# liu20050510/AA-CLIP-IQM

Hardware: AMD Instinct MI355X
Metric: images/sec ViT-L/14-336@518, batch 64 (higher is better)
Workload: dtype f16x2; 1 GPU; ViT-L/14-336 visual tower @518x518 with 4 tap layers (encode_image), batch 64 per GPU; global_batch=64, image=518x518, parallelism=dp1, input=batch resident in HBM, clip_weights=random fp32

## Files before the change

aa-clip-iqm_amd/aaclip_hip/_lib.py:

```python
from __future__ import annotations

import ctypes as C
import os
from typing import Optional

_HERE = os.path.dirname(os.path.abspath(__file__))
LIB_PATH = os.environ.get("AACLIP_LIB") or os.path.join(_HERE, "libaaclip_hip.so")
ABI_VERSION = 9

F32, F16, BF16, F16X2 = 0, 1, 2, 3
EXACT16_QKV, EXACT16_OUT, EXACT16_FC, EXACT16_PROJ, EXACT16_ADAPTER = 1, 2, 4, 8, 16
ACT_NONE, ACT_LEAKY, ACT_RELU = 0, 1, 2
EPI_BIAS, EPI_BIAS_GELU, EPI_BIAS_RESID, EPI_ACT_F32 = 0, 1, 2, 3
SEG_LOSS_FOCAL, SEG_LOSS_DICE0, SEG_LOSS_DICE1, SEG_LOSS_ALL = 1, 2, 4, 7

_vp, _i, _l, _f, _sz = C.c_void_p, C.c_int, C.c_long, C.c_float, C.c_size_t


class BlockWeights(C.Structure):
    _fields_ = [("struct_bytes", _sz)] + [(n, _vp) for n in (
        "ln1_w", "ln1_b", "qkv_w", "qkv_b", "out_w", "out_b", "ln2_w", "ln2_b",
        "fc_w", "fc_b", "proj_w", "proj_b", "adapter_w", "fc_w_fold", "fc_fold_s", "fc_fold_b",
        "qkv_w_fold", "qkv_fold_s", "qkv_fold_b")] + [("exact16", C.c_uint)]

# ... 11 lines not shown
    "aaclip_blocks": (_i, [_vp, C.POINTER(BlockWeights), _i, _f] + [_i] * 7 + [_vp, _sz, _vp]),
    "aaclip_blocks_to": (_i, [_vp, _vp, C.POINTER(BlockWeights), _i, _f] + [_i] * 7 + [_vp, _sz, _vp]),
    "aaclip_blocks_taps": (_i, [_vp, C.POINTER(_vp), C.POINTER(BlockWeights), _i, _f] + [_i] * 7 + [_vp, _sz, _vp]),
    "aaclip_tap_head": (_i, [_vp, _vp, _vp, _vp, _i, _vp, _vp, _vp] + [_i] * 5 + [_vp, _sz, _vp]),
    "aaclip_tap_head_keep_rows": (_i, [_vp, _vp, _vp, _vp, _i, _vp, _vp, _vp, _vp] + [_i] * 5 + [_vp, _sz, _vp]),
    "aaclip_det_head": (_i, [_vp, _vp, _vp, _vp, _i, _vp] + [_i] * 5 + [_vp, _sz, _vp]),
    "aaclip_anomaly_map": (_i, [C.POINTER(_vp), _i, _vp, _l, _vp, _i, _i, _i, _i, _i, _f, _vp, _sz, _vp]),
    "aaclip_similarity_map_train": (_i, [_vp, _vp, _l, _vp, _i, _i, _i, _i, _vp, _sz, _vp]),
    "aaclip_similarity_map_train_backward_workspace_bytes": (_sz, [_i, _i, _i]),
    "aaclip_similarity_map_train_backward": (_i, [_vp, _vp, _l, _vp, _vp, _vp, _vp, _i, _i, _i, _i, _vp, _sz, _vp]),
    "aaclip_seg_loss_workspace_bytes": (_sz, [_i]),
    "aaclip_seg_loss": (_i, [_vp, _l, _l, _vp, _i, _vp, _vp, _i, _l, _vp, _sz, _vp]),
    "aaclip_seg_loss_backward": (_i, [_vp, _l, _l, _vp, _i, _vp, _vp, _vp, _i, _l, _vp]),
    "aaclip_text_backward_workspace_bytes": (_sz, [_l, _i, _i]),
    "aaclip_gemm_wgrad": (_i, [_vp, _l, _vp, _l, _vp, _l, _i, _i, _vp, _sz, _vp]),
    "aaclip_attention_backward": (_i, [_vp, _vp, _vp, _i, _i, _i, _i, _f, _vp]),
    "aaclip_attention_backward_long_workspace_bytes": (_sz, [_i, _i, _i]),
    "aaclip_attention_backward_long": (_i, [_vp, _vp, _vp, _i, _i, _i, _i, _f, _vp, _sz, _vp]),
    "aaclip_layernorm_backward": (_i, [_vp, _vp, _vp, _vp, _vp, _l, _i, _f, _vp]),
    "aaclip_adapter_mix_backward": (_i, [_vp, _vp, _vp, _vp, _vp, _l, _i, _f, _vp]),
    "aaclip_block_backward": (_i, [_vp, C.POINTER(BlockWeights), C.POINTER(BlockWeights), _f] + [_i] * 6
                              + [_vp, _vp, _vp, _vp, _sz, _vp]),
    "aaclip_block_backward_long_workspace_bytes": (_sz, [_i, _i, _i, _i]),
    "aaclip_block_backward_long": (_i, [_vp, C.POINTER(BlockWeights), C.POINTER(BlockWeights), _f] + [_i] * 6
                                   + [_vp, _vp, _vp, _vp, _sz, _vp]),
    "aaclip_row_head_backward": (_i, [_vp] * 6 + [_i, _vp, _vp, _vp] + [_i] * 5 + [_vp, _sz, _vp]),
    "aaclip_text_embed": (_i, [_vp, _vp, _vp, _vp, _i, _i, _i, _i, _vp]),
    "aaclip_resample_ksize": (_i, [_i, _i]),
    "aaclip_resample_table": (_i, [_i, _i, _vp, _vp]),
    "aaclip_preprocess": (_i, [_vp, _i, _i, _i, _i, _vp, _vp, _vp, _vp, _vp, _vp, _vp]),
    "aaclip_row_head": (_i, [_vp, _vp, _vp, _vp, _vp, _i, _vp] + [_i] * 6 + [_vp, _sz, _vp]),
    "aaclip_layernorm": (_i, [_vp, _vp, _vp, _vp, _i, _l, _i, _f, _vp]),
    "aaclip_gemm": (_i, [_i, _i, _vp, _l, _vp, _vp, _vp, _l, _i, _i, _i, _i, _i, _f, _vp]),
    "aaclip_attention": (_i, [_i, _vp, _vp, _i, _i, _i, _i, _vp]),
    "aaclip_attention_log2q": (_i, [_i, _vp, _vp, _i, _i, _i, _i, _vp]),
    "aaclip_adapter_mix": (_i, [_vp, _vp, _l, _i, _f, _vp]),
    "aaclip_small_attention": (_i, [_i, _vp, _vp, _vp, _vp, _i, _i, _i, _i, _i, _f, _vp]),
    "aaclip_cross_rows_workspace_bytes": (_sz, [_i, _i, _i, _i]),
    "aaclip_cross_rows": (_i, [_i, _vp, _vp, _vp, _i, _i, _i, _i, _vp, _sz, _vp]),
    "aaclip_cross_rows_levels_workspace_bytes": (_sz, [_i, _i, _i, _i]),
    "aaclip_cross_rows_levels": (_i, [_i, _vp, _vp, _i, _vp, _i, _i, _i, _i, _i, _i, _l, _vp, _sz, _vp]),
    "aaclip_head_expand": (_i, [_i, _vp, _vp, _l, _i, _i, _f, _vp]),
    "aaclip_head_diag": (_i, [_vp, _vp, _l, _i, _i, _vp]),
    "aaclip_residual_layernorm": (_i, [_vp, _vp, _vp, _vp, _vp, _l, _i, _f, _vp]),
    "aaclip_combine3": (_i, [_vp, _vp, _vp, _f, _f, _f, _vp, _l, _vp]),
    "aaclip_linear_smallk": (_i, [_i, _vp, _vp, _vp, _vp, _l, _i, _i, _vp]),
    "aaclip_drop_cls_rows": (_i, [_i, _vp, _vp, _i, _i, _i, _i, _i, _vp]),
    "aaclip_iqm_map": (_i, [C.POINTER(_vp), _i, _vp, _vp, _vp, _i, _i, _i, _i, _f, _f, _vp, _sz, _vp]),
    "aaclip_set_gemm_variant": (_i, [_i]),
    "aaclip_profile_begin": (_i, [C.c_uint, _i]),
    "aaclip_profile_end": (_i, [C.POINTER(C.c_float), C.POINTER(C.c_int), _i]),
}

_lib: Optional[C.CDLL] = None


def load() -> C.CDLL:
    global _lib
    if _lib is None:
        if not os.path.exists(LIB_PATH):
            raise RuntimeError(
                f"{LIB_PATH} is missing: the AA-CLIP HIP extension has not been built "
                "(run `python -c 'import __graft_entry__ as g; g.build()'` or `make -C aa-clip-iqm_amd/csrc`). "
                "There is no PyTorch fallback for this path.")
        lib = C.CDLL(LIB_PATH)
        for name, (res, args) in SIGNATURES.items():
# ... 26 lines not shown
```

aa-clip-iqm_amd/csrc/capi.hip:

```cpp
#include <assert.h>
#include <stdio.h>
#include <stdlib.h>
#include <string.h>

#include "kernels.h"

using namespace aaclip;

static thread_local char g_err[512] = "";
static int g_ln_fold = 1;

static int fail(int code, const char* msg) {
  snprintf(g_err, sizeof(g_err), "%s", msg);
  return code;
}
#define REQUIRE(cond, msg) \
  do {                     \
    if (!(cond)) return fail(-1, msg); \
  } while (0)
#define REQUIRE_ALIGNED16(what, ...)                                            \
  do {                                                                          \
    const void* ptrs_[] = {__VA_ARGS__};                                        \
    for (const void* p_ : ptrs_)                                                \
      if ((uintptr_t)p_ & 15) return fail(-1, what ": pointers must be 16-byte aligned"); \
// ... 111 lines not shown
  l.big = l.narrow_bytes;
  l.big_bytes = wide > f32d ? wide : f32d;
  if (f32e > l.big_bytes) l.big_bytes = f32e;
  l.reserved = l.big + up256(l.big_bytes);
  l.x16 = l.reserved + up256((size_t)rows * 4);
  l.partials = l.x16 + up256((size_t)rows * D * es);
  l.rowab = l.partials + up256((size_t)rows * (D / 64 + 1) * 2 * 4);
  l.total = l.rowab + up256((size_t)rows * 2 * 4) + 4096;
  return l;
}

size_t aaclip_workspace_bytes(int dtype, long rows, int D, int F, int E) { return ws_layout(dtype, rows, D, F, E).total; }

int aaclip_layernorm(const float* x, const float* w, const float* b, void* out, int out_dtype, long rows, int D,
                     float eps, void* stream) {
  REQUIRE(x && w && b && out, "layernorm: null pointer");
  REQUIRE(dtype_ok(out_dtype), "layernorm: bad dtype");
  REQUIRE(rows > 0, "layernorm: rows must be positive");
  REQUIRE_ROW_WIDTH(D);
  launch_layernorm(out_dtype, x, w, b, out, rows, D, eps, (hipStream_t)stream);
  return finish("layernorm");
}

int aaclip_gemm(int dtype, int epi, const void* A, long lda, const void* W, const float* bias, void* out, long ldc,
                int M, int N, int K, int act, int scale_cols, float scale, void* stream) {
  REQUIRE(dtype_ok(dtype), "gemm: bad dtype");
  REQUIRE(epi >= AACLIP_EPI_BIAS && epi <= AACLIP_EPI_ACT_F32, "gemm: bad epilogue");
  GemmParams p = gemm_params(A, lda, W, bias, out, ldc, M, N, K);
  p.scale_cols = scale_cols; p.scale = scale; p.act = act;
  const char* m = gemm_check(dtype, epi, p);
  if (m) return fail(-1, m);
  launch_gemm(dtype, epi, p, (hipStream_t)stream);
  return finish("gemm");
}

static int attention_entry(int dtype, const void* qkv, void* ctx, int B, int L, int H, int causal, int log2q,
                           void* stream) {
  REQUIRE(qkv && ctx, "attention: null pointer");
  REQUIRE(B > 0 && L > 0 && H > 0, "attention: empty problem");
  REQUIRE(B <= 65535 && H <= 65535, "attention: grid limit");
  REQUIRE((long)L * 3 * 64 * H * 4 < (1L << 31), "attention: L * 3 * 64 * H * 4 must stay below 2^31 (32-bit row offsets)");
  REQUIRE((long)((L + 255) / 256) * H * B < (1L << 30), "attention: too many workgroups");
  launch_attention(dtype, qkv, ctx, B, L, H, causal, log2q, (hipStream_t)stream);
  return finish("attention");
}

int aaclip_attention(int dtype, const void* qkv, void* ctx, int B, int L, int H, int causal, void* stream) {
  REQUIRE(dtype_ok(dtype), "attention: bad dtype");
  return attention_entry(dtype, qkv, ctx, B, L, H, causal, 0, stream);
}

int aaclip_attention_log2q(int dtype, const void* qkv, void* ctx, int B, int L, int H, int causal, void* stream) {
  REQUIRE(dtype == AACLIP_F16 || dtype == AACLIP_BF16 || dtype == AACLIP_F16X2, "attention_log2q: 16-bit dtypes only");
  return attention_entry(dtype, qkv, ctx, B, L, H, causal, 1, stream);
}

int aaclip_adapter_mix(float* x, const float* a, long rows, int D, float weight, void* stream) {
  REQUIRE(x && a && rows > 0, "adapter_mix: bad arguments");
  REQUIRE_ROW_WIDTH(D);
  launch_adapter_mix(x, a, rows, D, weight, (hipStream_t)stream);
  return finish("adapter_mix");
}

int aaclip_small_attention(int kv_dtype, const float* q, const void* k, const void* v, float* out, int B, int nq, int Lk,
                           int H, int hd, float scale, void* stream) {
  REQUIRE(plain_dtype_ok(kv_dtype), "small_attention: bad dtype (fp32, fp16 or bf16)");
// ... 750 lines not shown
```

aa-clip-iqm_amd/csrc/common.h:

```cpp
#pragma once
#include <hip/hip_runtime.h>
#include <stdint.h>

typedef _Float16 f16;
typedef __bf16 bf16;

typedef _Float16 f16x8 __attribute__((ext_vector_type(8)));
typedef _Float16 f16x4 __attribute__((ext_vector_type(4)));
typedef __bf16 bf16x8 __attribute__((ext_vector_type(8)));
typedef __bf16 bf16x4 __attribute__((ext_vector_type(4)));
typedef short i16x4 __attribute__((ext_vector_type(4)));
typedef float f32x4 __attribute__((ext_vector_type(4)));
typedef float f32x16 __attribute__((ext_vector_type(16)));
typedef uint32_t u32x4 __attribute__((ext_vector_type(4)));
typedef uint32_t u32x2 __attribute__((ext_vector_type(2)));

#define AACLIP_DEV __device__ __forceinline__

template <typename T> struct Elem;
template <> struct Elem<f16> {
  typedef f16x8 vec8;
  typedef f16x4 vec4;
  static AACLIP_DEV f32x16 mma32(vec8 a, vec8 b, f32x16 c) {
    return __builtin_amdgcn_mfma_f32_32x32x16_f16(a, b, c, 0, 0, 0);
// ... 22 lines not shown
  c = __builtin_amdgcn_fmed3f(c * S, -448.f, 448.f);
  d = __builtin_amdgcn_fmed3f(d * S, -448.f, 448.f);
  int r = __builtin_amdgcn_cvt_pk_fp8_f32(a, b, 0, false);
  r = __builtin_amdgcn_cvt_pk_fp8_f32(c, d, r, true);
  return (uint32_t)r;
}
AACLIP_DEV void split8x4(const float (&v)[4], f16x4& hi, uint32_t& lo8, uint32_t& hi8) {
  float r[4];
#pragma unroll
  for (int j = 0; j < 4; ++j) {
    hi[j] = (f16)v[j];
    r[j] = v[j] - (float)hi[j];
  }
  lo8 = pack_e4m3x4<SPLIT8_ACT_LO_EXP>(r[0], r[1], r[2], r[3]);
  hi8 = pack_e4m3x4<SPLIT8_ACT_HI_EXP>(v[0], v[1], v[2], v[3]);
}
AACLIP_DEV void fp8_saturate_mode() { asm volatile("s_setreg_imm32_b32 hwreg(HW_REG_MODE, 23, 1), 1"); }
AACLIP_DEV void split8x4_sat(const float (&v)[4], f16x4& hi, uint32_t& lo8, uint32_t& hi8) {
  typedef short i16x2 __attribute__((ext_vector_type(2)));
  typedef float f32x4_ __attribute__((ext_vector_type(4)));
  const f32x4_ vv = {v[0], v[1], v[2], v[3]};
  hi = __builtin_convertvector(vv, f16x4);
  const f32x4_ r = vv - __builtin_convertvector(hi, f32x4_);
  constexpr float S_LO = 1.0f / (float)(1 << SPLIT8_ACT_LO_EXP);
  i16x2 a = {0, 0};
  a = __builtin_amdgcn_cvt_scalef32_pk_fp8_f32(a, r[0], r[1], S_LO, false);
  a = __builtin_amdgcn_cvt_scalef32_pk_fp8_f32(a, r[2], r[3], S_LO, true);
  lo8 = __builtin_bit_cast(uint32_t, a);
  static_assert(SPLIT8_ACT_HI_EXP == 0, "hi8 is the plain conversion");
  int b = __builtin_amdgcn_cvt_pk_fp8_f32(v[0], v[1], 0, false);
  b = __builtin_amdgcn_cvt_pk_fp8_f32(v[2], v[3], b, true);
  hi8 = (uint32_t)b;
}
template <int NP> AACLIP_DEV int vtile_off(int t, int K, int& kind) {
  if (NP == 0) { kind = 0; return t * 128; }
  int i, r;
  if (NP == 4) { i = t >> 2; r = t & 3; }
  else { i = (int)(((unsigned)t * 43691u) >> 17); r = t - 3 * i; }
  kind = r < 2 ? 0 : r - 1;
  return r < 2 ? (2 * i + r) * 128 : r * K + 128 * i;
}
template <int NP> AACLIP_DEV int vtile_count(int K) { return NP == 0 ? (K >> 6) : (NP == 4 ? (K >> 5) : 3 * (K >> 7)); }
AACLIP_DEV int vtile_scale_act(int kind) { return 127 - (kind == 1 ? SPLIT8_ACT_LO_EXP : SPLIT8_ACT_HI_EXP); }
AACLIP_DEV int vtile_scale_w(int kind) { return 127 - (kind == 1 ? SPLIT8_W_HI_EXP : SPLIT8_W_LO_EXP); }
typedef int i32x8 __attribute__((ext_vector_type(8)));
typedef int i32x4 __attribute__((ext_vector_type(4)));
AACLIP_DEV f32x4 mma_e4m3(f16x8 a0, f16x8 a1, f16x8 b0, f16x8 b1, f32x4 c, int scale_a, int scale_b) {
  const i32x4 x0 = __builtin_bit_cast(i32x4, a0), x1 = __builtin_bit_cast(i32x4, a1);
  const i32x4 y0 = __builtin_bit_cast(i32x4, b0), y1 = __builtin_bit_cast(i32x4, b1);
  const i32x8 a = __builtin_shufflevector(x0, x1, 0, 1, 2, 3, 4, 5, 6, 7);
  const i32x8 b = __builtin_shufflevector(y0, y1, 0, 1, 2, 3, 4, 5, 6, 7);
  return __builtin_amdgcn_mfma_scale_f32_16x16x128_f8f6f4(a, b, c, 0, 0, 0, scale_a, 0, scale_b);
}

AACLIP_DEV float wave_sum(float v) {
#pragma unroll
  for (int o = 32; o > 0; o >>= 1) v += __shfl_xor(v, o, 64);
  return v;
}
AACLIP_DEV float wave_max(float v) {
#pragma unroll
  for (int o = 32; o > 0; o >>= 1) v = fmaxf(v, __shfl_xor(v, o, 64));
  return v;
}

AACLIP_DEV int swz16(int rp) { return (rp & 0xA) | ((rp & 1) << 2) | ((rp >> 2) & 1); }
// ... 6 lines not shown

AACLIP_DEV void tile_src(int p, int& row, int& chunk) {
  int rp = p >> 4;
  int s = (p & 15) ^ swz16(rp & 15);
  row = rp * 2 + (s >> 3);
  chunk = s & 7;
}

typedef __attribute__((address_space(3))) void lds_void;
typedef const __attribute__((address_space(1))) void gbl_void;

AACLIP_DEV void glds16(const void* gsrc, void* lds_base) {
  __builtin_amdgcn_global_load_lds((gbl_void*)gsrc, (lds_void*)lds_base, 16, 0, 0);
}

template <typename P> AACLIP_DEV P* uniform_ptr(P* ptr) {
  const unsigned long long a = (unsigned long long)ptr;
  const unsigned lo = __builtin_amdgcn_readfirstlane((unsigned)a), hi = __builtin_amdgcn_readfirstlane((unsigned)(a >> 32));
  return (P*)(((unsigned long long)hi << 32) | lo);
}

AACLIP_DEV void wait_vm0() { asm volatile("s_waitcnt vmcnt(0)" ::: "memory"); }

AACLIP_DEV int xcd_remap(int id, int n) {
  int q = n >> 3, r = n & 7, x = id & 7, j = id >> 3;
  int base = (x < r) ? x * (q + 1) : r * (q + 1) + (x - r) * q;
  return base + j;
}

AACLIP_DEV float gelu_erf(float x) { return 0.5f * x * (1.0f + erff(x * 0.70710678118654752440f)); }
typedef float f32x2 __attribute__((ext_vector_type(2)));
AACLIP_DEV f32x2 fma2(f32x2 a, f32x2 b, f32x2 c) { return __builtin_elementwise_fma(a, b, c); }
AACLIP_DEV f32x2 splat2(float v) { return (f32x2){v, v}; }
AACLIP_DEV f32x2 gelu_fast2(f32x2 x) {
  f32x2 z = x * 0.70710678118654752440f;
  z[0] = __builtin_amdgcn_fmed3f(z[0], -3.2f, 3.2f);
  z[1] = __builtin_amdgcn_fmed3f(z[1], -3.2f, 3.2f);
  const f32x2 s = fma2(z * z, splat2(0.1953125f), splat2(-1.0f));
  f32x2 p = fma2(splat2(2.982273671e-03f), s, splat2(-7.046153473e-03f));
  p = fma2(p, s, splat2(7.957076705e-03f));
  p = fma2(p, s, splat2(-1.521942819e-02f));
  p = fma2(p, s, splat2(3.318292224e-02f));
  p = fma2(p, s, splat2(-5.471928813e-02f));
  p = fma2(p, s, splat2(8.062700147e-02f));
  p = fma2(p, s, splat2(-1.136467381e-01f));
  p = fma2(p, s, splat2(1.543549678e-01f));
  p = fma2(p, s, splat2(-2.173077339e-01f));
  p = fma2(p, s, splat2(4.413341836e-01f));
  const f32x2 hx = x * 0.5f;
  return fma2(hx, z * p, hx);
}
AACLIP_DEV float gelu_fast(float x) { return gelu_fast2((f32x2){x, x})[0]; }

AACLIP_DEV float leaky(float x) { return x >= 0.f ? x : 0.01f * x; }
```

aa-clip-iqm_amd/csrc/gemm256t.hip:

```cpp
#include "common.h"
#include "kernels.h"
#include "mma16.h"

namespace aaclip {

#define ST_OUT(ptr, v) __builtin_nontemporal_store(v, ptr)
#define LD_RESID(ptr) __builtin_nontemporal_load(ptr)
AACLIP_DEV float row16_sum(float x) {
  x += __builtin_bit_cast(float, __builtin_amdgcn_update_dpp(0, __builtin_bit_cast(int, x), 0x128, 0xF, 0xF, false));
  x += __builtin_bit_cast(float, __builtin_amdgcn_update_dpp(0, __builtin_bit_cast(int, x), 0x124, 0xF, 0xF, false));
  x += __builtin_bit_cast(float, __builtin_amdgcn_update_dpp(0, __builtin_bit_cast(int, x), 0x122, 0xF, 0xF, false));
  x += __builtin_bit_cast(float, __builtin_amdgcn_update_dpp(0, __builtin_bit_cast(int, x), 0x121, 0xF, 0xF, false));
  return x;
}
template <typename T, int EPI, bool SPLIT = false, bool QK8 = false, int NWC = 4, bool COMPACT = false>
AACLIP_DEV void epilogue256t(const GemmParams& p, f32x4 (&acc)[8][4], char* smem, int tm, int tn, int wave, int lane,
                             const f32x2* ab_pre = nullptr) {
  static_assert(!COMPACT || SPLIT, "the compact staging geometry exists for the split-operand epilogues");
  constexpr int STG = COMPACT ? 8192 : 16384;
  constexpr int SROWS = COMPACT ? 31 : 63;
  constexpr int SPL = COMPACT ? 4096 : 8192;
  typedef typename Elem<T>::vec4 vec4;
  asm volatile("" : "+v"(lane));
  const int c16 = lane & 15, q4 = lane >> 4;
  const int wr = NWC == 4 ? wave >> 2 : wave >> 1, wc = wave & (NWC - 1);
  const int m_base = tm * 256 + wr * 128, n_base = tn * (NWC * 64) + wc * 64;
  if (EPI == EPI_BIAS || EPI == EPI_BIAS_GELU) {
    __syncthreads();
    char* st = smem + wave * STG;
    const bool fold = p.row_ab != nullptr;
    f32x2 ab[8];
    if (fold) {
#pragma unroll
      for (int mi = 0; mi < 8; ++mi) {
        if (ab_pre) {
          ab[mi] = ab_pre[mi];
        } else {
          int row = m_base + mi * 16 + c16;
          row = row < p.M ? row : p.M - 1;
          ab[mi] = *(const f32x2*)(p.row_ab + 2L * row);
        }
      }
    }
    f32x4 bv[4], sv[4];
#pragma unroll
    for (int ni = 0; ni < 4; ++ni) {
      bv[ni] = *(const f32x4*)(p.bias + n_base + ni * 16 + 4 * q4);
      sv[ni] = (f32x4){0.f, 0.f, 0.f, 0.f};
      if (fold) sv[ni] = *(const f32x4*)(p.col_s + n_base + ni * 16 + 4 * q4);
    }
#pragma unroll
    for (int pass = 0; pass < 4; ++pass) {
#pragma unroll
      for (int ni = 0; ni < 4; ++ni) {
        const int nl = ni * 16 + 4 * q4;
#pragma unroll
        for (int hh = 0; hh < 2; ++hh) {
          const int mi = 2 * pass + hh;
          if (fold) {
#pragma unroll
            for (int j = 0; j < 4; ++j) acc[mi][ni][j] = fmaf(ab[mi][0], acc[mi][ni][j], ab[mi][1] * sv[ni][j]);
          }
          vec4 o, o2;
          float vv[4];
          if (EPI == EPI_BIAS_GELU) {
            f32x2 g0 = {acc[mi][ni][0] + bv[ni][0], acc[mi][ni][1] + bv[ni][1]};
            f32x2 g1 = {acc[mi][ni][2] + bv[ni][2], acc[mi][ni][3] + bv[ni][3]};
            g0 = gelu_fast2(g0);
            g1 = gelu_fast2(g1);
            vv[0] = g0[0]; vv[1] = g0[1]; vv[2] = g1[0]; vv[3] = g1[1];
          } else {
#pragma unroll
            for (int j = 0; j < 4; ++j) {
              float v = acc[mi][ni][j] + bv[ni][j];
              if (n_base + nl + j < p.scale_cols) v *= p.scale;
              vv[j] = v;
            }
          }
          const int m = mi * 16 + c16;
          if constexpr (SPLIT && EPI == EPI_BIAS) {
            if constexpr (QK8) {
              char* sp = st + (m & SROWS) * 128;
              if (n_base < p.out_qk8) {
                uint32_t l8, h8;
                split8x4_sat(vv, o, l8, h8);
                *(uint32_t*)(sp + SPL + (((nl >> 4) ^ (m & 7)) << 4) + (nl & 12)) = l8;
                *(uint32_t*)(sp + SPL + (((4 + (nl >> 4)) ^ (m & 7)) << 4) + (nl & 12)) = h8;
              } else {
#pragma unroll
                for (int j = 0; j < 4; ++j) o[j] = (f16)vv[j];
              }
              *(vec4*)(sp + ((((nl >> 3)) ^ (m & 7)) << 4) + (nl & 4) * 2) = o;
            } else {
#pragma unroll
            for (int j = 0; j < 4; ++j) {
              f16 hi, lo;
              split16(vv[j], hi, lo);
              o[j] = hi;
              o2[j] = lo;
            }
            char* sp = st + (m & SROWS) * 128 + ((((nl >> 3)) ^ (m & 7)) << 4) + (nl & 4) * 2;
            *(vec4*)sp = o;
            *(vec4*)(sp + SPL) = o2;
            }
          } else if constexpr (SPLIT) {
            uint32_t l8, h8;
            split8x4_sat(vv, o, l8, h8);
            char* sp = st + (m & SROWS) * 128;
            *(vec4*)(sp + ((((nl >> 3)) ^ (m & 7)) << 4) + (nl & 4) * 2) = o;
            *(uint32_t*)(sp + SPL + (((nl >> 4) ^ (m & 7)) << 4) + (nl & 12)) = l8;
            *(uint32_t*)(sp + SPL + (((4 + (nl >> 4)) ^ (m & 7)) << 4) + (nl & 12)) = h8;
          } else {
#pragma unroll
            for (int j = 0; j < 4; ++j) o[j] = from_float<T>(vv[j]);
            *(vec4*)(st + m * 128 + ((((nl >> 3)) ^ (m & 7)) << 4) + (nl & 4) * 2) = o;
          }
        }
      }
      {
        const int c = lane & 7, r8 = lane >> 3;
        u32x4 vh[4], vl[4];
#pragma unroll
        for (int k = 0; k < 4; ++k) {
          const int m = (4 * pass + k) * 8 + r8;
          if constexpr (SPLIT) {
            const char* sp = st + (m & SROWS) * 128 + ((c ^ (m & 7)) << 4);
            vh[k] = *(const u32x4*)sp;
            vl[k] = *(const u32x4*)(sp + SPL);
          } else {
            vh[k] = *(const u32x4*)(st + m * 128 + ((c ^ (m & 7)) << 4));
          }
        }
        char* const hb = (char*)((T*)p.out + (long)(m_base + r8) * p.ldc + n_base + c * 8);
        char* lb = hb;
        bool second = false;
        if constexpr (SPLIT) {
          char* const rb = (char*)((T*)p.out + (long)(m_base + r8) * p.ldc);
          if constexpr (EPI == EPI_BIAS) {
            if constexpr (QK8) {
              lb = rb + 2 * p.N + (n_base >> 6) * 128 + c * 16;
              second = n_base < p.out_qk8;
            } else {
              lb = rb + ((long)p.N + n_base + c * 8) * sizeof(T);
              second = true;
            }
          } else {
            lb = rb + 2 * p.N + (c >> 2) * p.N + n_base + (c & 3) * 16;
            second = c < 4 || !p.out_no_hi8;
          }
        }
        const long rstride = (long)p.ldc * sizeof(T) * 8;
        const bool inside = m_base + 128 <= p.M;
        if (inside) {
#pragma unroll
          for (int k = 0; k < 4; ++k) {
            const int it = 4 * pass + k;
            ST_OUT((u32x4*)(hb + it * rstride), vh[k]);
            if constexpr (SPLIT) {
              if (second) ST_OUT((u32x4*)(lb + it * rstride), vl[k]);
            }
          }
        } else {
#pragma unroll
          for (int k = 0; k < 4; ++k) {
            const int it = 4 * pass + k;
            if (m_base + it * 8 + r8 < p.M) {
              ST_OUT((u32x4*)(hb + it * rstride), vh[k]);
              if constexpr (SPLIT) {
                if (second) ST_OUT((u32x4*)(lb + it * rstride), vl[k]);
              }
            }
          }
        }
      }
    }
  } else {
    __syncthreads();
    char* st = smem + wave * STG;
    constexpr int PARTS = COMPACT ? 4 : 2;
    constexpr int PIT = 32 / PARTS, PMI = 8 / PARTS;
    const int cc = lane & 15, rr = lane >> 4;
    const int n0 = n_base + cc * 4;
    f32x4 bv = {0.f, 0.f, 0.f, 0.f};
    if (EPI == EPI_BIAS_RESID || (EPI == EPI_ACT_F32 && p.bias)) bv = *(const f32x4*)(p.bias + n0);
#pragma unroll
    for (int half = 0; half < PARTS; ++half) {
      f32x4 extra[PIT];
      long orow[PIT];
#pragma unroll
      for (int it = 0; it < PIT; ++it) {
        const int row = m_base + half * (4 * PIT) + it * 4 + rr;
        orow[it] = row;
        if (EPI == EPI_PATCH) {
          const int rc = row < p.M ? row : p.M - 1;
          const int b = rc / p.P, pi = rc - b * p.P;
          orow[it] = (long)b * p.L + 1 + pi;
          extra[it] = *(const f32x4*)(p.pos + (long)(1 + pi) * p.N + n0);
        } else if (EPI == EPI_BIAS_RESID) {
          const long rc = row < p.M ? row : p.M - 1;
          extra[it] = LD_RESID((const f32x4*)((p.resid ? p.resid : (const float*)p.out) + rc * p.ldc + n0));
        }
      }
#pragma unroll
      for (int mi = 0; mi < PMI; ++mi)
#pragma unroll
        for (int ni = 0; ni < 4; ++ni) {
          const int m = mi * 16 + c16;
// ... 645 lines not shown
#undef LD_M1
#undef LD_N
#undef MM
#undef MM8
#undef ROWT
#undef KTILE
  epilogue256t<T, EPI, NP != 0, QK8, 2>(p, acc, smem, tm, tn, wave, lane, fold_pre ? ab_pre : nullptr);
}

template <typename T, int NP>
static void launch_h(int epi, const GemmParams& p, hipStream_t s) {
  const int tiles_n = p.N / 128, tiles_m = (p.M + 255) / 256;
  int PN = 1;
  for (int c : {8, 6, 4, 3, 2}) if (tiles_n % c == 0) { PN = c; break; }
  const int patches_n = tiles_n / PN, PMx = 8;
  const int pm_x = (tiles_m + PMx - 1) / PMx;
  const int total_x = patches_n * pm_x;
  dim3 gx(((total_x + 7) / 8) * 8 * PMx * PN), b(256);
  const int stg = 1400;
  switch (epi) {
    case EPI_BIAS:
      if constexpr (NP != 0) {
        if (p.out_qk8) { hipLaunchKernelGGL((gemm16_256h_kernel<T, EPI_BIAS, NP, true>), gx, b, 0, s, p, PN, patches_n, total_x, PMx, stg); break; }
      }
      hipLaunchKernelGGL((gemm16_256h_kernel<T, EPI_BIAS, NP>), gx, b, 0, s, p, PN, patches_n, total_x, PMx, stg);
      break;
    case EPI_BIAS_GELU: hipLaunchKernelGGL((gemm16_256h_kernel<T, EPI_BIAS_GELU, NP>), gx, b, 0, s, p, PN, patches_n, total_x, PMx, stg); break;
    case EPI_BIAS_RESID: hipLaunchKernelGGL((gemm16_256h_kernel<T, EPI_BIAS_RESID, NP>), gx, b, 0, s, p, PN, patches_n, total_x, PMx, stg); break;
    case EPI_ACT_F32: hipLaunchKernelGGL((gemm16_256h_kernel<T, EPI_ACT_F32, NP>), gx, b, 0, s, p, PN, patches_n, total_x, PMx, stg); break;
    case EPI_PATCH: hipLaunchKernelGGL((gemm16_256h_kernel<T, EPI_PATCH, NP>), gx, b, 0, s, p, PN, patches_n, total_x, PMx, stg); break;
    default: set_launch_error("gemm: no 256-tile kernel for this epilogue");
  }
  if (p.out_qk8 && (epi != EPI_BIAS || NP == 0)) set_launch_error("gemm: out_qk8 goes with the bias epilogue of the split kernels only");
}

static void patch_shape(int tiles_n, int& PMx, int& PN) {
  PN = (tiles_n % 4 == 0) ? 4 : (tiles_n % 3 == 0) ? 3 : (tiles_n % 2 == 0) ? 2 : 1;
  PMx = 8;
}

static int walk_grid() {
  static int g = 0;
  if (g == 0) {
    int dev = 0, cus = 0;
    if (hipGetDevice(&dev) != hipSuccess || hipDeviceGetAttribute(&cus, hipDeviceAttributeMultiprocessorCount, dev) != hipSuccess || cus < 8)
      cus = 256;
    g = cus / 8 * 8;
  }
  return g;
}

template <int NP, bool WALK = false>
static void launch_split(int epi, const GemmParams& p, hipStream_t s) {
  const int tiles_n = p.N / 256, tiles_m = (p.M + 255) / 256;
  int PN, PMx;
  patch_shape(tiles_n, PMx, PN);
  const int patches_n = tiles_n / PN;
  const int pm_x = (tiles_m + PMx - 1) / PMx;
  const int total_x = patches_n * pm_x;
  const int vgrid = ((total_x + 7) / 8) * 8 * PMx * PN;
  dim3 gx(WALK ? (vgrid < walk_grid() ? vgrid : walk_grid()) : vgrid), b(512);
  switch (epi) {
    case EPI_BIAS:
      if (p.out_qk8) hipLaunchKernelGGL((gemm16_256x_kernel<f16, EPI_BIAS, NP, true, WALK>), gx, b, 0, s, p, PN, patches_n, total_x, PMx, vgrid);
      else hipLaunchKernelGGL((gemm16_256x_kernel<f16, EPI_BIAS, NP, false, WALK>), gx, b, 0, s, p, PN, patches_n, total_x, PMx, vgrid);
      break;
    case EPI_BIAS_GELU: hipLaunchKernelGGL((gemm16_256x_kernel<f16, EPI_BIAS_GELU, NP, false, WALK>), gx, b, 0, s, p, PN, patches_n, total_x, PMx, vgrid); break;
    case EPI_BIAS_RESID: hipLaunchKernelGGL((gemm16_256x_kernel<f16, EPI_BIAS_RESID, NP, false, WALK>), gx, b, 0, s, p, PN, patches_n, total_x, PMx, vgrid); break;
    case EPI_ACT_F32: hipLaunchKernelGGL((gemm16_256x_kernel<f16, EPI_ACT_F32, NP, false, WALK>), gx, b, 0, s, p, PN, patches_n, total_x, PMx, vgrid); break;
    case EPI_PATCH: hipLaunchKernelGGL((gemm16_256x_kernel<f16, EPI_PATCH, NP, false, WALK>), gx, b, 0, s, p, PN, patches_n, total_x, PMx, vgrid); break;
    default: set_launch_error("gemm: no 256-tile kernel for this epilogue");
  }
  if (p.out_qk8 && epi != EPI_BIAS) set_launch_error("gemm: out_qk8 goes with the bias epilogue only");
}

template <typename T>
static void launch_t(int epi, const GemmParams& p, hipStream_t s) {
  const int tiles_n = p.N / 256, tiles_m = (p.M + 255) / 256;
  int PN, PMx;
  patch_shape(tiles_n, PMx, PN);
  const int patches_n = tiles_n / PN, pm_x = (tiles_m + PMx - 1) / PMx;
  const int total_x = patches_n * pm_x;
  dim3 gx(((total_x + 7) / 8) * 8 * PMx * PN), b(512);
  if (((p.K >> 6) & 1) == 0) {
    switch (epi) {
      case EPI_BIAS: hipLaunchKernelGGL((gemm16_256x_kernel<T, EPI_BIAS>), gx, b, 0, s, p, PN, patches_n, total_x, PMx, 0); break;
      case EPI_BIAS_GELU: hipLaunchKernelGGL((gemm16_256x_kernel<T, EPI_BIAS_GELU>), gx, b, 0, s, p, PN, patches_n, total_x, PMx, 0); break;
      case EPI_BIAS_RESID: hipLaunchKernelGGL((gemm16_256x_kernel<T, EPI_BIAS_RESID>), gx, b, 0, s, p, PN, patches_n, total_x, PMx, 0); break;
      case EPI_ACT_F32: hipLaunchKernelGGL((gemm16_256x_kernel<T, EPI_ACT_F32>), gx, b, 0, s, p, PN, patches_n, total_x, PMx, 0); break;
      case EPI_PATCH: hipLaunchKernelGGL((gemm16_256x_kernel<T, EPI_PATCH>), gx, b, 0, s, p, PN, patches_n, total_x, PMx, 0); break;
      default: set_launch_error("gemm: no 256-tile kernel for this epilogue");
    }
    return;
  }
  switch (epi) {
    case EPI_BIAS: hipLaunchKernelGGL((gemm16_256v_kernel<T, EPI_BIAS>), gx, b, 0, s, p, PN, patches_n, total_x); break;
    case EPI_BIAS_GELU: hipLaunchKernelGGL((gemm16_256v_kernel<T, EPI_BIAS_GELU>), gx, b, 0, s, p, PN, patches_n, total_x); break;
    case EPI_BIAS_RESID: hipLaunchKernelGGL((gemm16_256v_kernel<T, EPI_BIAS_RESID>), gx, b, 0, s, p, PN, patches_n, total_x); break;
    case EPI_ACT_F32: hipLaunchKernelGGL((gemm16_256v_kernel<T, EPI_ACT_F32>), gx, b, 0, s, p, PN, patches_n, total_x); break;
    case EPI_PATCH: hipLaunchKernelGGL((gemm16_256v_kernel<T, EPI_PATCH>), gx, b, 0, s, p, PN, patches_n, total_x); break;
    default: set_launch_error("gemm: no 256-tile kernel for this epilogue");
  }
}

void launch_gemm256t(int dtype, int epi, const GemmParams& p, hipStream_t s, Gemm256Form form) {
  if (dtype == AACLIP_F16X2) {
// ... 24 lines not shown
```

include/aaclip.h:

```cpp
#ifndef AACLIP_H
#define AACLIP_H

#include <stddef.h>
#include <stdint.h>

#ifdef __cplusplus
extern "C" {
#endif

#define AACLIP_ABI_VERSION 9

enum { AACLIP_F32 = 0, AACLIP_F16 = 1, AACLIP_BF16 = 2, AACLIP_F16X2 = 3 };
enum { AACLIP_ACT_NONE = 0, AACLIP_ACT_LEAKY = 1, AACLIP_ACT_RELU = 2 };
enum { AACLIP_EPI_BIAS = 0, AACLIP_EPI_BIAS_GELU = 1, AACLIP_EPI_BIAS_RESID = 2, AACLIP_EPI_ACT_F32 = 3 };

int aaclip_version(void);
const char* aaclip_last_error(void);

size_t aaclip_workspace_bytes(int dtype, long rows, int D, int F, int E);

typedef struct aaclip_block_weights {
  size_t struct_bytes;
  const float* ln1_w;
  const float* ln1_b;
// ... 90 lines not shown
                          float* d_adapter_w, void* ws, size_t ws_bytes, void* stream);

size_t aaclip_block_backward_long_workspace_bytes(int B, int L, int D, int F);
int aaclip_block_backward_long(const float* x_in, const aaclip_block_weights* w, const aaclip_block_weights* wt,
                               float mix, int B, int L, int D, int H, int F, int attn_mode, const float* d_out,
                               float* d_in, float* d_adapter_w, void* ws, size_t ws_bytes, void* stream);

int aaclip_row_head_backward(const float* x, const int32_t* tokens, const float* ln_w, const float* ln_b,
                             const float* proj_w, const float* proj_wt, int act, const float* d_out, float* d_x,
                             float* d_proj_w, int n, int T, int D, int E, int mode, void* ws, size_t ws_bytes,
                             void* stream);

int aaclip_resample_ksize(int in_size, int out_size);
int aaclip_resample_table(int in_size, int out_size, int32_t* bounds, int32_t* coefs);
int aaclip_preprocess(const uint8_t* src, int B, int Hs, int Ws, int S, const int32_t* hbounds, const int32_t* hcoefs,
                      const int32_t* vbounds, const int32_t* vcoefs, const float* lut, float* out, void* stream);

int aaclip_text_embed(const int32_t* tokens, const float* table, const float* pos, float* x, int n, int T, int D,
                      int vocab, void* stream);

int aaclip_row_head(const float* x, const int32_t* tokens, const float* ln_w, const float* ln_b, const void* proj_w,
                    int act, float* out, int n, int T, int D, int E, int mode, int dtype, void* ws, size_t ws_bytes,
                    void* stream);

int aaclip_profile_begin(unsigned tag_mask, int capacity);
int aaclip_profile_end(float* ms, int* tags, int max_n);

int aaclip_set_gemm_variant(int v);

int aaclip_layernorm(const float* x, const float* w, const float* b, void* out, int out_dtype, long rows, int D,
                     float eps, void* stream);
int aaclip_gemm(int dtype, int epi, const void* A, long lda, const void* W, const float* bias, void* out, long ldc,
                int M, int N, int K, int act, int scale_cols, float scale, void* stream);
int aaclip_attention(int dtype, const void* qkv, void* ctx, int B, int L, int H, int causal, void* stream);
int aaclip_attention_log2q(int dtype, const void* qkv, void* ctx, int B, int L, int H, int causal, void* stream);
int aaclip_adapter_mix(float* x, const float* a, long rows, int D, float weight, void* stream);


size_t aaclip_cross_rows_workspace_bytes(int B, int R, int Lk, int Dk);
int aaclip_cross_rows(int x_dtype, const float* qt, const void* x, float* out, int B, int R, int Lk, int Dk, void* ws,
                      size_t ws_bytes, void* stream);
size_t aaclip_cross_rows_levels_workspace_bytes(int B, int nseg, int Lk, int Dk);
int aaclip_cross_rows_levels(int x_dtype, const float* qt, const void* const* x, int nseg, float* out, int B, int R,
                             int rows_per_image, int row0, int Lk, int Dk, long ldx, void* ws, size_t ws_bytes,
                             void* stream);
int aaclip_head_expand(int dtype, const float* q, void* qm, long rows, int H, int D, float scale, void* stream);
int aaclip_head_diag(const float* full, float* ctx, long rows, int H, int D, void* stream);
int aaclip_small_attention(int kv_dtype, const float* q, const void* k, const void* v, float* out, int B, int nq, int Lk,
                           int H, int hd, float scale, void* stream);
int aaclip_residual_layernorm(const float* a, const float* b, const float* w, const float* bias, float* out, long rows,
                              int D, float eps, void* stream);
int aaclip_combine3(const float* a, const float* b, const float* c, float wa, float wb, float wc, float* out, long n,
                    void* stream);
int aaclip_linear_smallk(int out_dtype, const float* x, const float* W, const float* bias, void* y, long R, int N, int K,
                         void* stream);
int aaclip_drop_cls_rows(int dtype, const void* src, void* dst, int B, int L, int E, int rows_per_image, int row_off,
                         void* stream);
int aaclip_iqm_map(const float* const* seg, int NL, const float* queries, const float* base, float* out, int B, int g,
                   int E, int S, float w_base, float w_iqm, void* ws, size_t ws_bytes, void* stream);

#ifdef __cplusplus
}
#endif
#endif
```

Before: 542.1 images/s.

## Restructure split-GEMM epilogue: hoist QK8 branch, interleave GELU, cheaper fp8 split

Reworks the 256-tile GEMM epilogue for split (f16x2) outputs. The per-tile QK8 branch is hoisted into a compile-time-specialized lambda so each tile runs one branch-free path. GELU is evaluated on two vectors at a time to interleave the polynomial chains. The fp8 hi/lo split uses v_fma_mix and scaled fp8 conversion, and column scaling is precomputed per column group. It also adds wave-level fences in place of implicit ordering, a new C API entry that forces the 256-tile walk path for testing, and guards against the LayerNorm fold on split operands. The risks are more code and register pressure from the duplicated specialization, and subtle numeric changes in the fp8 split.

```diff
diff --git a/aa-clip-iqm_amd/aaclip_hip/_lib.py b/aa-clip-iqm_amd/aaclip_hip/_lib.py
--- a/aa-clip-iqm_amd/aaclip_hip/_lib.py
+++ b/aa-clip-iqm_amd/aaclip_hip/_lib.py
@@ -67,6 +67,7 @@
     "aaclip_row_head": (_i, [_vp, _vp, _vp, _vp, _vp, _i, _vp] + [_i] * 6 + [_vp, _sz, _vp]),
     "aaclip_layernorm": (_i, [_vp, _vp, _vp, _vp, _i, _l, _i, _f, _vp]),
     "aaclip_gemm": (_i, [_i, _i, _vp, _l, _vp, _vp, _vp, _l, _i, _i, _i, _i, _i, _f, _vp]),
+    "aaclip_gemm_split_tile256": (_i, [_i, _vp, _l, _vp, _vp, _vp, _l, _i, _i, _i, _i, _f, _i, _i, _vp]),
     "aaclip_attention": (_i, [_i, _vp, _vp, _i, _i, _i, _i, _vp]),
     "aaclip_attention_log2q": (_i, [_i, _vp, _vp, _i, _i, _i, _i, _vp]),
     "aaclip_adapter_mix": (_i, [_vp, _vp, _l, _i, _f, _vp]),
diff --git a/aa-clip-iqm_amd/csrc/capi.hip b/aa-clip-iqm_amd/csrc/capi.hip
--- a/aa-clip-iqm_amd/csrc/capi.hip
+++ b/aa-clip-iqm_amd/csrc/capi.hip
@@ -167,6 +167,23 @@
   if (m) return fail(-1, m);
   launch_gemm(dtype, epi, p, (hipStream_t)stream);
   return finish("gemm");
+}
+
+int aaclip_gemm_split_tile256(int epi, const void* A, long lda, const void* W, const float* bias, void* out, long ldc,
+                              int M, int N, int K, int scale_cols, float scale, int out_qk8, int out_no_hi8,
+                              void* stream) {
+  REQUIRE(epi == AACLIP_EPI_BIAS || epi == AACLIP_EPI_BIAS_GELU, "gemm_split_tile256: bias or bias + GELU epilogue");
+  REQUIRE(out_qk8 >= 0 && out_qk8 % 64 == 0 && out_qk8 <= N, "gemm_split_tile256: out_qk8 must be whole heads within N");
+  REQUIRE(out_qk8 == 0 || epi == AACLIP_EPI_BIAS, "gemm_split_tile256: out_qk8 goes with the bias epilogue");
+  REQUIRE(ldc >= (out_qk8 ? N + out_qk8 : 2L * N), "gemm_split_tile256: ldc too small for the output rows");
+  GemmParams p = gemm_params(A, lda, W, bias, out, ldc, M, N, K);
+  p.scale_cols = scale_cols; p.scale = scale;
+  p.out_qk8 = out_qk8; p.out_no_hi8 = out_no_hi8 ? 1 : 0;
+  const char* m = gemm_check(AACLIP_F16X2, epi, p);
+  if (m) return fail(-1, m);
+  REQUIRE(gemm256_applicable(AACLIP_F16X2, p), "gemm_split_tile256: shape not accepted by the 256-tile kernel");
+  launch_gemm256t(AACLIP_F16X2, epi, p, (hipStream_t)stream, GEMM256_WALK);
+  return finish("gemm_split_tile256");
 }
 
 static int attention_entry(int dtype, const void* qkv, void* ctx, int B, int L, int H, int causal, int log2q,
diff --git a/aa-clip-iqm_amd/csrc/common.h b/aa-clip-iqm_amd/csrc/common.h
--- a/aa-clip-iqm_amd/csrc/common.h
+++ b/aa-clip-iqm_amd/csrc/common.h
@@ -78,6 +78,30 @@
   b = __builtin_amdgcn_cvt_pk_fp8_f32(v[2], v[3], b, true);
   hi8 = (uint32_t)b;
 }
+AACLIP_DEV f16x4 split8_hi(const float (&v)[4]) {
+  typedef float f32x4_ __attribute__((ext_vector_type(4)));
+  const f32x4_ vv = {v[0], v[1], v[2], v[3]};
+  return __builtin_convertvector(vv, f16x4);
+}
+AACLIP_DEV void split8_planes(const float (&v)[4], f16x4 hi, uint32_t& lo8, uint32_t& hi8) {
+  typedef short i16x2 __attribute__((ext_vector_type(2)));
+  const u32x2 hw = __builtin_bit_cast(u32x2, hi);
+  float r[4];
+#pragma unroll
+  for (int j = 0; j < 4; ++j) {
+    if (j & 1) asm("v_fma_mix_f32 %0, %1, -1.0, %2 op_sel:[1,0,0] op_sel_hi:[1,0,0]" : "=v"(r[j]) : "v"(hw[j >> 1]), "v"(v[j]));
+    else asm("v_fma_mix_f32 %0, %1, -1.0, %2 op_sel_hi:[1,0,0]" : "=v"(r[j]) : "v"(hw[j >> 1]), "v"(v[j]));
+  }
+  constexpr float S_LO = 1.0f / (float)(1 << SPLIT8_ACT_LO_EXP);
+  i16x2 a = __builtin_bit_cast(i16x2, r[0]);
+  a = __builtin_amdgcn_cvt_scalef32_pk_fp8_f32(a, r[0], r[1], S_LO, false);
+  a = __builtin_amdgcn_cvt_scalef32_pk_fp8_f32(a, r[2], r[3], S_LO, true);
+  lo8 = __builtin_bit_cast(uint32_t, a);
+  static_assert(SPLIT8_ACT_HI_EXP == 0, "hi8 is the plain conversion");
+  int b = __builtin_amdgcn_cvt_pk_fp8_f32(v[0], v[1], __builtin_bit_cast(int, v[0]), false);
+  b = __builtin_amdgcn_cvt_pk_fp8_f32(v[2], v[3], b, true);
+  hi8 = (uint32_t)b;
+}
 template <int NP> AACLIP_DEV int vtile_off(int t, int K, int& kind) {
   if (NP == 0) { kind = 0; return t * 128; }
   int i, r;
@@ -150,23 +174,34 @@
 typedef float f32x2 __attribute__((ext_vector_type(2)));
 AACLIP_DEV f32x2 fma2(f32x2 a, f32x2 b, f32x2 c) { return __builtin_elementwise_fma(a, b, c); }
 AACLIP_DEV f32x2 splat2(float v) { return (f32x2){v, v}; }
+template <int NP> AACLIP_DEV void gelu_fast2n(f32x2 (&x)[NP]) {
+  constexpr float C[10] = {-7.046153473e-03f, 7.957076705e-03f, -1.521942819e-02f, 3.318292224e-02f, -5.471928813e-02f,
+                           8.062700147e-02f, -1.136467381e-01f, 1.543549678e-01f, -2.173077339e-01f, 4.413341836e-01f};
+  f32x2 z[NP], s[NP], p[NP];
+#pragma unroll
+  for (int u = 0; u < NP; ++u) {
+    z[u] = x[u] * 0.70710678118654752440f;
+    z[u][0] = __builtin_amdgcn_fmed3f(z[u][0], -3.2f, 3.2f);
+    z[u][1] = __builtin_amdgcn_fmed3f(z[u][1], -3.2f, 3.2f);
+  }
+#pragma unroll
+  for (int u = 0; u < NP; ++u) s[u] = fma2(z[u] * z[u], splat2(0.1953125f), splat2(-1.0f));
+#pragma unroll
+  for (int u = 0; u < NP; ++u) p[u] = fma2(splat2(2.982273671e-03f), s[u], splat2(C[0]));
+#pragma unroll
+  for (int k = 1; k < 10; ++k)
+#pragma unroll
+    for (int u = 0; u < NP; ++u) p[u] = fma2(p[u], s[u], splat2(C[k]));
+#pragma unroll
+  for (int u = 0; u < NP; ++u) {
+    const f32x2 hx = x[u] * 0.5f;
+    x[u] = fma2(hx, z[u] * p[u], hx);
+  }
+}
 AACLIP_DEV f32x2 gelu_fast2(f32x2 x) {
-  f32x2 z = x * 0.70710678118654752440f;
-  z[0] = __builtin_amdgcn_fmed3f(z[0], -3.2f, 3.2f);
-  z[1] = __builtin_amdgcn_fmed3f(z[1], -3.2f, 3.2f);
-  const f32x2 s = fma2(z * z, splat2(0.1953125f), splat2(-1.0f));
-  f32x2 p = fma2(splat2(2.982273671e-03f), s, splat2(-7.046153473e-03f));
-  p = fma2(p, s, splat2(7.957076705e-03f));
-  p = fma2(p, s, splat2(-1.521942819e-02f));
-  p = fma2(p, s, splat2(3.318292224e-02f));
-  p = fma2(p, s, splat2(-5.471928813e-02f));
-  p = fma2(p, s, splat2(8.062700147e-02f));
-  p = fma2(p, s, splat2(-1.136467381e-01f));
-  p = fma2(p, s, splat2(1.543549678e-01f));
-  p = fma2(p, s, splat2(-2.173077339e-01f));
-  p = fma2(p, s, splat2(4.413341836e-01f));
-  const f32x2 hx = x * 0.5f;
-  return fma2(hx, z * p, hx);
+  f32x2 v[1] = {x};
+  gelu_fast2n<1>(v);
+  return v[0];
 }
 AACLIP_DEV float gelu_fast(float x) { return gelu_fast2((f32x2){x, x})[0]; }
 
diff --git a/aa-clip-iqm_amd/csrc/gemm256t.hip b/aa-clip-iqm_amd/csrc/gemm256t.hip
--- a/aa-clip-iqm_amd/csrc/gemm256t.hip
+++ b/aa-clip-iqm_amd/csrc/gemm256t.hip
@@ -13,6 +13,7 @@
   x += __builtin_bit_cast(float, __builtin_amdgcn_update_dpp(0, __builtin_bit_cast(int, x), 0x121, 0xF, 0xF, false));
   return x;
 }
+template <bool B> struct BoolC { static constexpr bool value = B; };
 template <typename T, int EPI, bool SPLIT = false, bool QK8 = false, int NWC = 4, bool COMPACT = false>
 AACLIP_DEV void epilogue256t(const GemmParams& p, f32x4 (&acc)[8][4], char* smem, int tm, int tn, int wave, int lane,
                              const f32x2* ab_pre = nullptr) {
@@ -28,7 +29,7 @@
   if (EPI == EPI_BIAS || EPI == EPI_BIAS_GELU) {
     __syncthreads();
     char* st = smem + wave * STG;
-    const bool fold = p.row_ab != nullptr;
+    const bool fold = !SPLIT && p.row_ab != nullptr;
     f32x2 ab[8];
     if (fold) {
 #pragma unroll
@@ -43,136 +44,150 @@
       }
     }
     f32x4 bv[4], sv[4];
+    float qs[4];
 #pragma unroll
     for (int ni = 0; ni < 4; ++ni) {
       bv[ni] = *(const f32x4*)(p.bias + n_base + ni * 16 + 4 * q4);
       sv[ni] = (f32x4){0.f, 0.f, 0.f, 0.f};
       if (fold) sv[ni] = *(const f32x4*)(p.col_s + n_base + ni * 16 + 4 * q4);
-    }
-#pragma unroll
-    for (int pass = 0; pass < 4; ++pass) {
-#pragma unroll
-      for (int ni = 0; ni < 4; ++ni) {
-        const int nl = ni * 16 + 4 * q4;
-#pragma unroll
-        for (int hh = 0; hh < 2; ++hh) {
-          const int mi = 2 * pass + hh;
-          if (fold) {
-#pragma unroll
-            for (int j = 0; j < 4; ++j) acc[mi][ni][j] = fmaf(ab[mi][0], acc[mi][ni][j], ab[mi][1] * sv[ni][j]);
-          }
-          vec4 o, o2;
-          float vv[4];
-          if (EPI == EPI_BIAS_GELU) {
-            f32x2 g0 = {acc[mi][ni][0] + bv[ni][0], acc[mi][ni][1] + bv[ni][1]};
-            f32x2 g1 = {acc[mi][ni][2] + bv[ni][2], acc[mi][ni][3] + bv[ni][3]};
-            g0 = gelu_fast2(g0);
-            g1 = gelu_fast2(g1);
-            vv[0] = g0[0]; vv[1] = g0[1]; vv[2] = g1[0]; vv[3] = g1[1];
-          } else {
-#pragma unroll
-            for (int j = 0; j < 4; ++j) {
-              float v = acc[mi][ni][j] + bv[ni][j];
-              if (n_base + nl + j < p.scale_cols) v *= p.scale;
-              vv[j] = v;
+      qs[ni] = n_base + ni * 16 + 4 * q4 < p.scale_cols ? p.scale : 1.0f;
+    }
+    auto passes = [&](auto rec_c) __attribute__((always_inline)) {
+      constexpr bool REC = decltype(rec_c)::value;
+#pragma unroll
+      for (int pass = 0; pass < 4; ++pass) {
+#pragma unroll
+        for (int ni = 0; ni < 4; ++ni) {
+          const int nl = ni * 16 + 4 * q4;
+#pragma unroll
+          for (int hh = 0; hh < 2; ++hh) {
+            const int mi = 2 * pass + hh;
+            if (fold) {
+#pragma unroll
+              for (int j = 0; j < 4; ++j) acc[mi][ni][j] = fmaf(ab[mi][0], acc[mi][ni][j], ab[mi][1] * sv[ni][j]);
+            }
+            vec4 o, o2;
+            float vv[4];
+            if (EPI == EPI_BIAS_GELU) {
+              f32x2 g[2] = {{acc[mi][ni][0] + bv[ni][0], acc[mi][ni][1] + bv[ni][1]},
+                            {acc[mi][ni][2] + bv[ni][2], acc[mi][ni][3] + bv[ni][3]}};
+              gelu_fast2n<2>(g);
+              vv[0] = g[0][0]; vv[1] = g[0][1]; vv[2] = g[1][0]; vv[3] = g[1][1];
+            } else {
+#pragma unroll
+              for (int j = 0; j < 4; ++j) {
+                float v = acc[mi][ni][j] + bv[ni][j];
+                if constexpr (SPLIT) v *= qs[ni];
+                else if (n_base + nl + j < p.scale_cols) v *= p.scale;
+                vv[j] = v;
+              }
+            }
+            const int m = mi * 16 + c16;
+            if constexpr (SPLIT && EPI == EPI_BIAS) {
+              if constexpr (QK8) {
+                char* sp = st + (m & SROWS) * 128;
+                o = split8_hi(vv);
+                if constexpr (REC) {
+                  uint32_t l8, h8;
+                  split8_planes(vv, o, l8, h8);
+                  *(uint32_t*)(sp + SPL + (((nl >> 4) ^ (m & 7)) << 4) + (nl & 12)) = l8;
+                  *(uint32_t*)(sp + SPL + (((4 + (nl >> 4)) ^ (m & 7)) << 4) + (nl & 12)) = h8;
+                }
+                *(vec4*)(sp + ((((nl >> 3)) ^ (m & 7)) << 4) + (nl & 4) * 2) = o;
+              } else {
+#pragma unroll
+              for (int j = 0; j < 4; ++j) {
+                f16 hi, lo;
+                split16(vv[j], hi, lo);
+                o[j] = hi;
+                o2[j] = lo;
+              }
+              char* sp = st + (m & SROWS) * 128 + ((((nl >> 3)) ^ (m & 7)) << 4) + (nl & 4) * 2;
+              *(vec4*)sp = o;
+              *(vec4*)(sp + SPL) = o2;
+              }
+            } else if constexpr (SPLIT) {
+              uint32_t l8, h8;
+              o = split8_hi(vv);
+              split8_planes(vv, o, l8, h8);
+              char* sp = st + (m & SROWS) * 128;
+              *(vec4*)(sp + ((((nl >> 3)) ^ (m & 7)) << 4) + (nl & 4) * 2) = o;
+              *(uint32_t*)(sp + SPL + (((nl >> 4) ^ (m & 7)) << 4) + (nl & 12)) = l8;
+              *(uint32_t*)(sp + SPL + (((4 + (nl >> 4)) ^ (m & 7)) << 4) + (nl & 12)) = h8;
+            } else {
+#pragma unroll
+              for (int j = 0; j < 4; ++j) o[j] = from_float<T>(vv[j]);
+              *(vec4*)(st + m * 128 + ((((nl >> 3)) ^ (m & 7)) << 4) + (nl & 4) * 2) = o;
             }
           }
-          const int m = mi * 16 + c16;
-          if constexpr (SPLIT && EPI == EPI_BIAS) {
-            if constexpr (QK8) {
-              char* sp = st + (m & SROWS) * 128;
-              if (n_base < p.out_qk8) {
-                uint32_t l8, h8;
-                split8x4_sat(vv, o, l8, h8);
-                *(uint32_t*)(sp + SPL + (((nl >> 4) ^ (m & 7)) << 4) + (nl & 12)) = l8;
-                *(uint32_t*)(sp + SPL + (((4 + (nl >> 4)) ^ (m & 7)) << 4) + (nl & 12)) = h8;
-              } else {
-#pragma unroll
-                for (int j = 0; j < 4; ++j) o[j] = (f16)vv[j];
-              }
-              *(vec4*)(sp + ((((nl >> 3)) ^ (m & 7)) << 4) + (nl & 4) * 2) = o;
+        }
+        __builtin_amdgcn_fence(__ATOMIC_RELEASE, "wavefront");
+        __builtin_amdgcn_wave_barrier();
+        {
+          const int c = lane & 7, r8 = lane >> 3;
+          u32x4 vh[4], vl[4];
+#pragma unroll
+          for (int k = 0; k < 4; ++k) {
+            const int m = (4 * pass + k) * 8 + r8;
+            if constexpr (SPLIT) {
+              const char* sp = st + (m & SROWS) * 128 + ((c ^ (m & 7)) << 4);
+              vh[k] = *(const u32x4*)sp;
+              vl[k] = *(const u32x4*)(sp + SPL);
             } else {
-#pragma unroll
-            for (int j = 0; j < 4; ++j) {
-              f16 hi, lo;
-              split16(vv[j], hi, lo);
-              o[j] = hi;
-              o2[j] = lo;
-            }
-            char* sp = st + (m & SROWS) * 128 + ((((nl >> 3)) ^ (m & 7)) << 4) + (nl & 4) * 2;
-            *(vec4*)sp = o;
-            *(vec4*)(sp + SPL) = o2;
-            }
-          } else if constexpr (SPLIT) {
-            uint32_t l8, h8;
-            split8x4_sat(vv, o, l8, h8);
-            char* sp = st + (m & SROWS) * 128;
-            *(vec4*)(sp + ((((nl >> 3)) ^ (m & 7)) << 4) + (nl & 4) * 2) = o;
-            *(uint32_t*)(sp + SPL + (((nl >> 4) ^ (m & 7)) << 4) + (nl & 12)) = l8;
-            *(uint32_t*)(sp + SPL + (((4 + (nl >> 4)) ^ (m & 7)) << 4) + (nl & 12)) = h8;
-          } else {
-#pragma unroll
-            for (int j = 0; j < 4; ++j) o[j] = from_float<T>(vv[j]);
-            *(vec4*)(st + m * 128 + ((((nl >> 3)) ^ (m & 7)) << 4) + (nl & 4) * 2) = o;
-          }
-        }
-      }
-      {
-        const int c = lane & 7, r8 = lane >> 3;
-        u32x4 vh[4], vl[4];
-#pragma unroll
-        for (int k = 0; k < 4; ++k) {
-          const int m = (4 * pass + k) * 8 + r8;
-          if constexpr (SPLIT) {
-            const char* sp = st + (m & SROWS) * 128 + ((c ^ (m & 7)) << 4);
-            vh[k] = *(const u32x4*)sp;
-            vl[k] = *(const u32x4*)(sp + SPL);
-          } else {
-            vh[k] = *(const u32x4*)(st + m * 128 + ((c ^ (m & 7)) << 4));
-          }
-        }
-        char* const hb = (char*)((T*)p.out + (long)(m_base + r8) * p.ldc + n_base + c * 8);
-        char* lb = hb;
-        bool second = false;
-        if constexpr (SPLIT) {
-          char* const rb = (char*)((T*)p.out + (long)(m_base + r8) * p.ldc);
-          if constexpr (EPI == EPI_BIAS) {
-            if constexpr (QK8) {
-              lb = rb + 2 * p.N + (n_base >> 6) * 128 + c * 16;
-              second = n_base < p.out_qk8;
-            } else {
-              lb = rb + ((long)p.N + n_base + c * 8) * sizeof(T);
-              second = true;
-            }
-          } else {
-            lb = rb + 2 * p.N + (c >> 2) * p.N + n_base + (c & 3) * 16;
-            second = c < 4 || !p.out_no_hi8;
-          }
-        }
-        const long rstride = (long)p.ldc * sizeof(T) * 8;
-        const bool inside = m_base + 128 <= p.M;
-        if (inside) {
-#pragma unroll
-          for (int k = 0; k < 4; ++k) {
-            const int it = 4 * pass + k;
-            ST_OUT((u32x4*)(hb + it * rstride), vh[k]);
-            if constexpr (SPLIT) {
-              if (second) ST_OUT((u32x4*)(lb + it * rstride), vl[k]);
+              vh[k] = *(const u32x4*)(st + m * 128 + ((c ^ (m & 7)) << 4));
             }
           }
-        } else {
-#pragma unroll
-          for (int k = 0; k < 4; ++k) {
-            const int it = 4 * pass + k;
-            if (m_base + it * 8 + r8 < p.M) {
+          __builtin_amdgcn_fence(__ATOMIC_ACQUIRE, "wavefront");
+          __builtin_amdgcn_wave_barrier();
+          char* const hb = (char*)((T*)p.out + (long)(m_base + r8) * p.ldc + n_base + c * 8);
+          char* lb = hb;
+          bool second = false;
+          if constexpr (SPLIT) {
+            char* const rb = (char*)((T*)p.out + (long)(m_base + r8) * p.ldc);
+            if constexpr (EPI == EPI_BIAS) {
+              if constexpr (QK8) {
+                lb = rb + 2 * p.N + (n_base >> 6) * 128 + c * 16;
+                second = REC;
+              } else {
+                lb = rb + ((long)p.N + n_base + c * 8) * sizeof(T);
+                second = true;
+              }
+            } else {
+              lb = rb + 2 * p.N + (c >> 2) * p.N + n_base + (c & 3) * 16;
+              second = c < 4 || !p.out_no_hi8;
+            }
+          }
+          const long rstride = (long)p.ldc * sizeof(T) * 8;
+          const bool inside = m_base + 128 <= p.M;
+          if (inside) {
+#pragma unroll
+            for (int k = 0; k < 4; ++k) {
+              const int it = 4 * pass + k;
               ST_OUT((u32x4*)(hb + it * rstride), vh[k]);
               if constexpr (SPLIT) {
                 if (second) ST_OUT((u32x4*)(lb + it * rstride), vl[k]);
               }
             }
+          } else {
+#pragma unroll
+            for (int k = 0; k < 4; ++k) {
+              const int it = 4 * pass + k;
+              if (m_base + it * 8 + r8 < p.M) {
+                ST_OUT((u32x4*)(hb + it * rstride), vh[k]);
+                if constexpr (SPLIT) {
+                  if (second) ST_OUT((u32x4*)(lb + it * rstride), vl[k]);
+                }
+              }
+            }
           }
         }
       }
+    };
+    if constexpr (SPLIT && EPI == EPI_BIAS && QK8) {
+      if (n_base < p.out_qk8) passes(BoolC<true>{});
+      else passes(BoolC<false>{});
+    } else {
+      passes(BoolC<false>{});
     }
   } else {
     __syncthreads();
@@ -884,6 +899,7 @@
     default: set_launch_error("gemm: no 256-tile kernel for this epilogue");
   }
   if (p.out_qk8 && (epi != EPI_BIAS || NP == 0)) set_launch_error("gemm: out_qk8 goes with the bias epilogue of the split kernels only");
+  if (p.row_ab && NP != 0) set_launch_error("gemm: the LayerNorm fold (row_ab) exists for plain 16-bit operands only");
 }
 
 static void patch_shape(int tiles_n, int& PMx, int& PN) {
@@ -924,6 +940,7 @@
     default: set_launch_error("gemm: no 256-tile kernel for this epilogue");
   }
   if (p.out_qk8 && epi != EPI_BIAS) set_launch_error("gemm: out_qk8 goes with the bias epilogue only");
+  if (p.row_ab) set_launch_error("gemm: the LayerNorm fold (row_ab) exists for plain 16-bit operands only");
 }
 
 template <typename T>
diff --git a/include/aaclip.h b/include/aaclip.h
--- a/include/aaclip.h
+++ b/include/aaclip.h
@@ -146,6 +146,9 @@
                      float eps, void* stream);
 int aaclip_gemm(int dtype, int epi, const void* A, long lda, const void* W, const float* bias, void* out, long ldc,
                 int M, int N, int K, int act, int scale_cols, float scale, void* stream);
+int aaclip_gemm_split_tile256(int epi, const void* A, long lda, const void* W, const float* bias, void* out, long ldc,
+                              int M, int N, int K, int scale_cols, float scale, int out_qk8, int out_no_hi8,
+                              void* stream);
 int aaclip_attention(int dtype, const void* qkv, void* ctx, int B, int L, int H, int causal, void* stream);
 int aaclip_attention_log2q(int dtype, const void* qkv, void* ctx, int B, int L, int H, int causal, void* stream);
 int aaclip_adapter_mix(float* x, const float* a, long rows, int D, float weight, void* stream);
```

After: 547.2 images/s (median of 6 runs). No clear change (+1.0%).
